# ymingxie/PARQ

Measured on AMD Instinct MI355X. Metric: decoder-iterations/sec (10 views, 256 queries, d=256), higher is better.
Workload: dtype f32 (cross-attention scores: fp16 hi.hi + MX-fp8 e4m3 cross terms; P V: fp16 probabilities and values with a self-consistent normaliser; fp32 accumulation — 4e-6..1.5e-5 from float64 at the outputs on the reference's fixtures, the reference's own fp32 run: 6e-5..1.4e-4; guarded: rows on too few keys

## Files before the change

parq_amd/csrc/api.hip:

```cpp
#include "../../include/parq_hip.h"
#include "common.hpp"

#include <cmath>
#include <cstdarg>
#include <cstdio>
#include <cstring>
#include <map>
#include <string>
#include <vector>

using namespace parq;

namespace {
constexpr float kPeakyL = 256.f;

thread_local char g_err[512] = "";

int fail(int code, const char* fmt, ...) {
    va_list ap;
    va_start(ap, fmt);
    vsnprintf(g_err, sizeof(g_err), fmt, ap);
    va_end(ap);
    return code;
}
// ... 434 lines not shown
            HIPCHK(half(L.cross_in_w, C, C, nullptr, A + L.n1_b, A + L.cross_in_b));
            HIPCHK(half(L.cross_out_w, C, C));
            HIPCHK(half(L.lin1_w, F, C, A + L.n2_w, A + L.n2_b, A + L.lin1_b)); HIPCHK(half(L.lin2_w, C, F));
        }
        HIPCHK(half(ar.pe2_w, C, C));
        if (c->nl == 1) HIPCHK(half(ar.heads1_w, c->NH1, C, A + ar.layers[0].n3_w, A + ar.layers[0].n3_b, A + ar.heads1_b));
        else HIPCHK(half(ar.heads1_w, c->NH1, C));
        HIPCHK(half(ar.heads2_w, C, C)); HIPCHK(half(ar.heads2_w + C * C, C, C));
    }
    c->derived_valid = true;
    return PARQ_OK;
}

struct ShardIO { int mask = 7; const float* in = nullptr; float* out = nullptr; int nranks = 1; };

int do_iterate(parq_ctx* c, const parq_scene* sc, float* wsp, const Workspace& ws, int layer_num, const float* ref,
               bool emb_valid, const parq_outputs* o, float* ref_out, hipStream_t s, int64_t shift = 0,
               float* emb_next = nullptr, bool train = false, const ShardIO& sh = ShardIO(), int64_t captured_row0 = -1,
               bool last_of_forward = false) {
    const void* const* ind = captured_row0 >= 0 ? reinterpret_cast<const void* const*>(wsp + ws.ind) : nullptr;
    const float* cam_in = ind ? wsp + ws.cam : sc->camera;
    const int64_t row0 = captured_row0 >= 0 ? captured_row0 : 0;
    float* wi = wsp + shift;
    const bool sharded = sh.mask != 7;
    if (!emb_next) emb_next = wi + ws.emb;
    const float dp = train ? c->drop_p : 0.f;
    const float* A = c->arena;
    const Arena& ar = c->ar;
    if (!train && !c->derived_valid) { const int rc = build_derived_weights(c, s); if (rc) return rc; }
    const float* TP = train ? nullptr : A + ar.tile_off;
    const bool h3 = !train && ar.half_off >= 0 && c->attn_mode != 0 && chain_h3_on();
    auto halfw = [&](LinearArgs& la, int64_t off, int fold = 0) {
        if (h3) {
            la.Wh = A + ar.half_off + off; la.wh_scale = A + ar.hscale_off + hscale_slot(off);
// ... 16 lines not shown
        return a;
    };
    auto cross_q_args = [&](bool fold) {
        LinearArgs a = lin(wi + ws.xa, C, A + L.cross_in_w, C, A + (fold ? L.cross_q_b2 : L.cross_in_b), wi + ws.qc, C, M, C, C);
        a.ln_gamma = A + L.n1_w; a.ln_beta = A + L.n1_b; a.ln_stats_out = wi + ws.ln1; a.norm_eps = eps;
        a.ldx2 = C; a.x2_ncols = C; a.Wp = TP ? TP + L.cross_in_w : nullptr; halfw(a, L.cross_in_w, 2);
        if (fold) { a.X2 = wi + ws.pe_h; a.W2 = A + L.cross_q_w2; a.W2p = TP ? TP + L.cross_q_w2 : nullptr; }
        else a.X2 = wi + ws.pos;
        return a;
    };
    static const bool fold_off = [] { const char* e = dev_env("PARQ_FOLD_POS"); return e && e[0] == '0'; }();
    const bool fold_pos = !train && !fold_off && chain_linear_supported(self_in_args(true), 1) && chain_linear_supported(cross_q_args(true), 1);
    static const int seams = [] { const char* e = dev_env("PARQ_FUSE_SEAMS"); return e ? atoi(e) : 1; }();
    const bool seam_ok = !train && !sharded && fold_pos && C == 256 && TP != nullptr && M % 16 == 0 && c->seam_fusion;

    if (sh.mask & 1) {
    if (!emb_valid) { Prof p(c, s, PARQ_PROF_OTHER); HIPCHK(launch_posemb(ref, A + ar.dim_t, M, wi + ws.emb, s)); }
    LinearArgs pe1 = lin(wi + ws.emb, 384, A + ar.pe0_w, 384, A + ar.pe0_b, wi + ws.pe_h, C, M, C, 384);
    pe1.relu = 1; pe1.Wp = TP ? TP + ar.pe0_w : nullptr;
    float* sample_out = sharded ? sh.out : wi + ws.tgt;
    float* sample_cnt = sharded ? sh.out + (int64_t)M * C : nullptr;
    static const bool fuse_off = [] { const char* e = dev_env("PARQ_FUSE_PE1_SAMPLE"); return e && e[0] == '0'; }();
    bool fused = false;
    if (!train && !fuse_off && !c->profiling) {
        const hipError_t e = launch_pe1_sample(pe1, sc->tokens, reinterpret_cast<const double*>(wsp + ws.T_cl), cam_in, ref, c->sb, B, sc->V,
                                               sc->h, sc->w, C, Q, sample_out, o->coord_pos, gn1, B * 8 * kGnSlots, sample_cnt, s, ind, row0 * 3,
                                               c->tok_type);
        if (e == hipSuccess) fused = true;
        else if (e != hipErrorNotSupported) return fail(PARQ_ERR_HIP, "launch_pe1_sample failed: %s", hipGetErrorString(e));
    }
    {
        Prof p(c, s, PARQ_PROF_LINEAR);
        if (!fused) HIPCHK(launch_linear(pe1, 1, s));
        if (!fold_pos) {
            LinearArgs a = lin(wi + ws.pe_h, C, A + ar.pe2_w, C, A + ar.pe2_b, wi + ws.pos, C, M, C, C);
            a.Wp = TP ? TP + ar.pe2_w : nullptr; halfw(a, ar.pe2_w);
            HIPCHK(launch_linear(a, 1, s));
        }
    }
    if (!fused) {
        Prof p(c, s, PARQ_PROF_PROJECT_SAMPLE);
        HIPCHK(launch_project_sample_f64(sc->tokens, reinterpret_cast<const double*>(wsp + ws.T_cl), cam_in, ref, c->sb,
                                         B, sc->V, sc->h, sc->w, C, Q, sample_out, o->coord_pos, gn1, B * 8 * kGnSlots, s, sample_cnt, ind, row0 * 3,
                                         c->tok_type));
    }
    if (sharded) HIPCHK(launch_shard_range_flag(c->cache_mode() && c->kind() == kF16 ? reinterpret_cast<const int*>(wsp + ws.flags) : nullptr,
                                                sh.out + (int64_t)M * C + M, s));
    }
    if (sh.mask & 2) {
    if (sharded) {
        Prof p(c, s, PARQ_PROF_PROJECT_SAMPLE);
        HIPCHK(launch_sample_finalize(sh.in, sh.in + (int64_t)M * C, M, C, wi + ws.tgt, s, sh.in + (int64_t)M * C + M,
                                      c->cache_mode() && c->kind() == kF16 ? reinterpret_cast<int*>(wsp + ws.flags) : nullptr));
    }
    {
        Prof p(c, s, PARQ_PROF_LINEAR);
        LinearArgs a = self_in_args(fold_pos);
        HIPCHK(launch_linear(a, 1, s));
    }
    FlashArgs fa;
    memset(&fa, 0, sizeof(fa));
    fa.B = B; fa.H = H; fa.Lq = Q; fa.dh = dh;
    fa.out = wi + ws.sa; fa.out_batch = (int64_t)Q * C; fa.out_row = C;
    {
        Prof p(c, s, PARQ_PROF_SELF_ATTN);
        static const bool self_one = [] { const char* e = dev_env("PARQ_SELF_ONE_LAUNCH"); return !(e && e[0] == '0'); }();
        if (dh <= 64 || (self_one && (dh == 128 || dh == 256) && Q <= 1024)) {
            HIPCHK(launch_self_attn(wi + ws.qkv, 3 * C, B, H, Q, dh, wi + ws.sa, C, s, train ? wi + ws.lse_s : nullptr, dp,
                                    c->site_seed(layer_num, 0)));
        } else {
            fa.q = wi + ws.qkv;         fa.q_batch = (int64_t)Q * 3 * C; fa.q_head = dh; fa.q_row = 3 * C;
            fa.k = wi + ws.qkv + C;     fa.k_batch = fa.q_batch; fa.k_head = dh; fa.k_row = 3 * C;
            fa.v = wi + ws.qkv + 2 * C; fa.v_batch = fa.q_batch; fa.v_head = dh; fa.v_row = 3 * C;
            fa.Lk = Q; fa.nsplit = ws.self_split;
            const int64_t lp = flash_lq_pad(Q);
            fa.o_part = wsp + ws.flash;
            fa.m_part = fa.o_part + (int64_t)B * H * fa.nsplit * dh * lp;
            fa.l_part = fa.m_part + (int64_t)B * H * fa.nsplit * lp;
            fa.lse = train ? wi + ws.lse_s : nullptr;
            fa.drop_p = dp; fa.drop_seed = c->site_seed(layer_num, 0);
            HIPCHK(launch_flash(fa, s));
            HIPCHK(launch_flash_merge(fa, s));
        }
    }
    fa.out = sharded ? sh.out : wi + ws.attn;
    fa.lse = sharded ? sh.out + (int64_t)M * C : (train ? wi + ws.lse_c : nullptr);
    fa.drop_p = dp; fa.drop_seed = c->site_seed(layer_num, 2);
    bool fused_q = false;
    {
        Prof p(c, s, PARQ_PROF_LINEAR);
        LinearArgs a = lin(wi + ws.sa, C, A + L.self_out_w, C, A + L.self_out_b, wi + ws.xa, C, M, C, C);
        a.R = wi + ws.tgt; a.ldr = C; a.Wp = TP ? TP + L.self_out_w : nullptr; halfw(a, L.self_out_w);
        a.drop_p = dp; a.drop_seed = c->site_seed(layer_num, 1);
        if (seam_ok && (seams & 1)) {
            a.lnp_out = reinterpret_cast<double*>(wi + ws.lnp1);
            a.lnp_flags = reinterpret_cast<unsigned*>(wsp + ws.seam_flags);
            a.lnp_epoch = c->next_epoch();
            SeamArgs q;
            memset(&q, 0, sizeof(q));
            q.X1 = wi + ws.sa; q.ldx1 = C; q.W1p = TP + L.qo_w;
            q.X2 = wi + ws.tgt; q.ldx2 = C; q.W2p = TP + L.qg_w;
            q.X3 = wi + ws.pe_h; q.ldx3 = C; q.W3p = TP + L.cross_q_w2;
            q.b1 = A + L.qu_b; q.srow = A + L.q_s; q.b2 = A + L.qv_b;
            q.Y = wi + ws.qc; q.ldy = C; q.M = M; q.N = C;
            q.part = a.lnp_out; q.flags = a.lnp_flags; q.epoch = a.lnp_epoch; q.nparts = C / 64; q.width = C; q.eps = eps;
            q.ln_out = wi + ws.ln1;
            q.err = reinterpret_cast<int*>(wsp + ws.flags);
            const hipError_t e = launch_seam_q(a, q, s);
            if (e == hipSuccess) fused_q = true;
            else if (e != hipErrorNotSupported) return fail(PARQ_ERR_HIP, "launch_seam_q failed: %s", hipGetErrorString(e));
            a.lnp_out = nullptr; a.lnp_flags = nullptr;
        }
        if (!fused_q) {
            HIPCHK(launch_linear(a, 1, s));
            a = cross_q_args(fold_pos);
            HIPCHK(launch_linear(a, 1, s));
        }
    }
    bool merged = false;
    {
        Prof p(c, s, PARQ_PROF_CROSS_ATTN);
        fa.q = wi + ws.qc; fa.q_batch = (int64_t)Q * C; fa.q_head = dh; fa.q_row = C;
        fa.Lk = (int)N; fa.nsplit = ws.cross_split;
        const int alt_phase = [] { const char* e = dev_env("PARQ_FLASH_ALT_PHASE"); return e && e[0] == '1' ? 1 : 0; }();
        fa.flags = ((layer_num + alt_phase) & 1) ? 2 : 0;
        const int64_t lp = flash_lq_pad(Q);
        fa.o_part = wsp + ws.flash;
        fa.m_part = fa.o_part + (int64_t)B * H * fa.nsplit * dh * lp;
        fa.l_part = fa.m_part + (int64_t)B * H * fa.nsplit * lp;
        if (c->cache_mode()) {
            const char* cache = reinterpret_cast<const char*>(wsp + ws.kvc) + (size_t)li * kvsplit_cache_bytes(B, c->vheads(), (int)N, c->terms());
// ... 29 lines not shown
                    { Prof pm(c, s, PARQ_PROF_MERGE); HIPCHK(launch_flash_merge(f8, s)); HIPCHK(launch_flash_merge(f3, s)); }
                    merged = true;
                }
            }
            else {
                if (c->attn_mode == 4 && !train && !sharded && H <= 16 && dh == 64) fa.head_min = reinterpret_cast<int*>(wsp + ws.flags) + 32;
                HIPCHK(launch_flash_split(fa, cache, s, c->terms(), c->kind()));
            }
        } else {
            const float* kv = wsp + ws.kv + (int64_t)li * B * 2 * N * C;
            fa.k = kv;                       fa.k_batch = 2 * N * C; fa.k_head = N * dh; fa.k_row = dh;
            fa.v = kv + (int64_t)H * N * dh; fa.v_batch = 2 * N * C; fa.v_head = N * dh; fa.v_row = dh;
            HIPCHK(launch_flash(fa, s));
        }
    }
    if (!merged) { Prof p(c, s, PARQ_PROF_MERGE); HIPCHK(launch_flash_merge(fa, s)); }
    }
    if (!(sh.mask & 4)) return PARQ_OK;
    if (sharded) {
        Prof p(c, s, PARQ_PROF_MERGE);
        const int64_t rec = (int64_t)M * C + (int64_t)B * H * flash_lq_pad(Q);
        HIPCHK(launch_attn_combine(sh.in, sh.nranks, rec, B, H, Q, flash_lq_pad(Q), dh, wi + ws.attn, s));
    }
    {
        Prof p(c, s, PARQ_PROF_LINEAR);
        LinearArgs a = lin(wi + ws.attn, C, A + L.cross_out_w, C, A + L.cross_out_b, wi + ws.xb, C, M, C, C);
        a.R = wi + ws.xa; a.ldr = C; a.rln_stats = wi + ws.ln1; a.rln_gamma = A + L.n1_w; a.rln_beta = A + L.n1_b; a.Wp = TP ? TP + L.cross_out_w : nullptr; halfw(a, L.cross_out_w);
        a.drop_p = dp; a.drop_seed = c->site_seed(layer_num, 3);
        if (last_of_forward && c->progress_word != nullptr) {
            a.pub_flags = reinterpret_cast<const int*>(wsp + ws.flags);
            a.pub_mirror = c->range_mirror; a.pub_word = c->progress_word;
            a.pub_epoch = reinterpret_cast<const int*>(wsp + ws.ind) + 14;
            a.pub_mask = (c->cache_mode() && c->kind() == kF16) ? ~0 : 4;
            a.pub_peaky = c->terms_for(N, false) == 8 ? 1 : 0;
        }
        HIPCHK(launch_linear(a, 1, s));
        a = lin(wi + ws.xb, C, A + L.lin1_w, C, A + L.lin1_b, wi + ws.ffn, F, M, F, C);
        a.ln_gamma = A + L.n2_w; a.ln_beta = A + L.n2_b; a.ln_stats_out = wi + ws.ln2; a.norm_eps = eps;
        a.relu = 1; a.Wp = TP ? TP + L.lin1_w : nullptr; halfw(a, L.lin1_w, 1);
        a.drop_p = dp; a.drop_seed = c->site_seed(layer_num, 4);
        HIPCHK(launch_linear(a, 1, s));
        a = lin(wi + ws.ffn, F, A + L.lin2_w, F, A + L.lin2_b, wi + ws.xc, C, M, C, F);
        a.R = wi + ws.xb; a.ldr = C; a.rln_stats = wi + ws.ln2; a.rln_gamma = A + L.n2_w; a.rln_beta = A + L.n2_b; a.Wp = TP ? TP + L.lin2_w : nullptr; halfw(a, L.lin2_w);
        a.drop_p = dp; a.drop_seed = c->site_seed(layer_num, 5);
        HIPCHK(launch_linear(a, 1, s));
        const int NH1 = c->NH1;
        a = lin(wi + ws.xc, C, A + ar.heads1_w, C, A + ar.heads1_b, wi + ws.h1, NH1, M, NH1, C);
        a.ln_gamma = A + L.n3_w; a.ln_beta = A + L.n3_b; a.norm_eps = eps;
        if (train) a.ln_stats_out = wi + ws.ln3;
        if (NH1 % 16 == 0) { a.Wp = TP ? TP + ar.heads1_w : nullptr; halfw(a, ar.heads1_w, c->nl == 1 ? 1 : 0); }
        a.gn_out_sums = gn1; a.gn_out_ncols = 2 * C; a.gn_out_group_cols = C; a.gn_out_rows_per_scene = Q; a.gn_out_ngroups = 2;
        HIPCHK(launch_linear(a, 1, s));
        if (train && c->deterministic) HIPCHK(launch_gn_moments_det(wi + ws.h1, NH1, C, 2, Q, B, gn1, s));
        a = lin(wi + ws.h1, NH1, A + ar.heads2_w, C, nullptr, wi + ws.h2, 2 * C, M, C, C);
        a.gn_sums = gn1; a.gn_gamma = A + ar.gn1_g; a.gn_beta = A + ar.gn1_b; a.norm_eps = eps;
        a.gn_rows_per_scene = Q; a.gn_ngroups = 2;
        a.gX = C; a.gW = (int64_t)C * C; a.gY = C; a.gGamma = C; a.Wp = TP ? TP + ar.heads2_w : nullptr; halfw(a, ar.heads2_w);
        a.gn_out_sums = gn2; a.gn_out_ncols = C; a.gn_out_group_cols = C; a.gn_out_rows_per_scene = Q; a.gn_out_ngroups = 2;
        HIPCHK(launch_linear(a, 2, s));
        if (train && c->deterministic) HIPCHK(launch_gn_moments_det(wi + ws.h2, 2 * C, C, 2, Q, B, gn2, s));
    }
    {
        Prof p(c, s, PARQ_PROF_OTHER);
        BoxDecodeArgs d;
        memset(&d, 0, sizeof(d));
        d.h1 = wi + ws.h1 + 2 * C; d.ld1 = c->NH1;
        d.h2 = wi + ws.h2; d.ld2 = 2 * C;
        d.gn_sums = gn2; d.gn_gamma = A + ar.gn2_g; d.gn_beta = A + ar.gn2_b;
        d.w3 = A + ar.heads3_w; d.b3 = A + ar.heads3_b; d.C = C; d.rows_per_scene = Q; d.eps = eps;
        d.ref = ref; d.mean_sizes = A + ar.mean_sizes; d.n_mean = c->cfg.num_mean_sizes; d.dim_t = A + ar.dim_t;
        d.poison = reinterpret_cast<const int*>(wsp + ws.flags);
        d.poison_mask = (c->cache_mode() && c->kind() == kF16) ? ~0 : 4;
        d.poison_mirror = (last_of_forward && c->progress_word != nullptr) ? nullptr : c->range_mirror;
        d.peaky = (!sharded && c->terms_for(N, train, train && bwd_reads_cache(c, ws)) == 8) ? reinterpret_cast<const int*>(wsp + ws.flags) + 1 : nullptr;
        d.peaky_poison = c->peaky_poison;
        d.sb = c->sb; d.M = M; d.ncls = c->ncls;
        d.logits = o->pred_logits; d.center = o->center_unnormalized; d.size = o->size_unnormalized;
        d.rot = o->ortho6d; d.prob = o->sem_cls_prob; d.ref_next = ref_out; d.emb_next = emb_next;
        d.ind = ind; d.out_row0 = row0;
        HIPCHK(launch_box_decode(d, s));
    }
    return PARQ_OK;
}


struct BwdIO {
    const float* g_logits; const float* g_center; const float* g_size; const float* g_rot;
    const float* center; const float* size;
};

int do_backward_transposes(parq_ctx* c, float* wsp, const Workspace& ws, int li, hipStream_t s) {
    const float* A = c->arena;
    const Arena& ar = c->ar;
    const LayerW& L = ar.layers[li];
    const int C = c->C, F = c->F, NH1 = c->NH1;
// ... 504 lines not shown
    const int64_t M = (int64_t)scene->B * h->Q;
    float* ra = wsp + ws.ref;
    float* rb = wsp + ws.ref_next;
    for (int k = 0; k < h->I; ++k) {
        parq_outputs o;
        memset(&o, 0, sizeof(o));
        if (!captured) {
            o.pred_logits = outs->pred_logits + k * M * h->ncls;
            o.center_unnormalized = outs->center_unnormalized + k * M * 3;
            o.size_unnormalized = outs->size_unnormalized + k * M * 3;
            o.ortho6d = outs->ortho6d + k * M * 6;
            o.sem_cls_prob = outs->sem_cls_prob + k * M * h->ncls;
            o.coord_pos = outs->coord_pos + k * M * 3;
        }
        const int rc = do_iterate(h, scene, wsp, ws, k, ra, true, &o, rb, s, 0, nullptr, false, ShardIO(),
                                  captured ? k * M : -1, k + 1 == h->I);
        if (rc) return rc;
        float* t = ra; ra = rb; rb = t;
    }
    h->ref_state = 0;
    h->prepared = false;
    return PARQ_OK;
}

static int forward_checks(parq_handle h, const parq_scene* scene, void* workspace, size_t workspace_bytes, const parq_outputs* outs, Workspace* ws) {
    if (!h || !workspace) return fail(PARQ_ERR_ARG, "NULL argument");
    if (!h->packed) return fail(PARQ_ERR_STATE, "parq_pack_weights must be called first");
    int rc = check_scene(h, scene);
    if (rc) return rc;
    rc = check_outs(outs);
    if (rc) return rc;
// ... 887 lines not shown
```

parq_amd/csrc/chain.hip:

```cpp
#include "common.hpp"
#include "sample_body.hpp"

namespace parq {

namespace {

typedef float f32x4v __attribute__((ext_vector_type(4)));

enum : int { kProNone = 0, kProLN = 1, kProGN = 2 };
enum : int { kResNone = 0, kResPlain = 1, kResLN = 2 };

template <int K, int NT, int PRO, int ADD2, bool BIAS, bool RELU, int RES, bool GNOUT, int NWV = 4, bool LNP = false>
__device__ __forceinline__ void chain_tile(const LinearArgs& a, const int block_x, const int block_y) {
    if (block_x == 0 && block_y == 0) publish_progress(a);
    static_assert(K % (16 * NWV) == 0 && NT >= 1 && NT <= 4 && (NWV == 4 || NWV == 8), "tile shape");
    constexpr int NCH = K / (16 * NWV);
    constexpr int CS = 16 * NWV;
    __shared__ __attribute__((aligned(16))) float red[NWV * NT * 4 * 64];
    __shared__ float lnred[NWV * 16 * 2];

    const int g = block_y;
    const int ntn = a.N / (16 * NT);
    int n0, m0;
    if (a.tile_map == 0) {
// ... 65 lines not shown
    }
    const int et = wave % NT;
    const int erow = lane >> 2, ec = (lane & 3) * 4;
    const int om = m0 + erow, on = n0 + et * 16 + ec;
    f32x4v e_bias = {0.f, 0.f, 0.f, 0.f}, e_r = {0.f, 0.f, 0.f, 0.f}, e_rg = {1.f, 1.f, 1.f, 1.f}, e_rb = {0.f, 0.f, 0.f, 0.f};
    float rmean = 0.f, rrstd = 1.f;
    if constexpr (BIAS) e_bias = *reinterpret_cast<const f32x4v*>(a.bias + g * a.gBias + on);
    if constexpr (RES != kResNone) e_r = *reinterpret_cast<const f32x4v*>(a.R + (int64_t)om * a.ldr + on);
    if constexpr (RES == kResLN) {
        e_rg = *reinterpret_cast<const f32x4v*>(a.rln_gamma + on);
        e_rb = *reinterpret_cast<const f32x4v*>(a.rln_beta + on);
        rmean = a.rln_stats[(int64_t)om * 2 + 0];
        rrstd = a.rln_stats[(int64_t)om * 2 + 1];
    }
    __builtin_amdgcn_sched_barrier(0);

    if constexpr (PRO == kProLN) {
        float sm = 0.f, sq = 0.f;
#pragma unroll
        for (int c = 0; c < NCH; ++c)
#pragma unroll
            for (int e = 0; e < 4; ++e) {
                const float d = av[c][e] - shift;
                sm += d;
                sq += d * d;
            }
        sm += __shfl_xor(sm, 16); sq += __shfl_xor(sq, 16);
        sm += __shfl_xor(sm, 32); sq += __shfl_xor(sq, 32);
        if (kq == 0) { lnred[(wave * 16 + li) * 2 + 0] = sm; lnred[(wave * 16 + li) * 2 + 1] = sq; }
        lds_barrier();
// ... 46 lines not shown
    if constexpr (ADD2 == 2) {
        if (n0 < a.x2_ncols) {
#pragma unroll
            for (int c = 0; c < NCH; ++c)
#pragma unroll
                for (int e = 0; e < 4; ++e)
#pragma unroll
                    for (int t = 0; t < NT; ++t) acc[t] = __builtin_amdgcn_mfma_f32_16x16x4f32(x2v[c][e], b2v[t][c][e], acc[t], 0, 0, 0);
        }
    }
#pragma unroll
    for (int t = 0; t < NT; ++t)
#pragma unroll
        for (int r = 0; r < 4; ++r) red[((wave * NT + t) * 4 + r) * 64 + lane] = acc[t][r];
    lds_barrier();
    if (wave >= NT) return;

    const int src = (wave * 4 + (erow & 3)) * 64 + (erow >> 2) * 16 + ec;
    f32x4v sum = *reinterpret_cast<const f32x4v*>(&red[src]);
#pragma unroll
    for (int w = 1; w < NWV; ++w) sum += *reinterpret_cast<const f32x4v*>(&red[src + w * NT * 256]);
    f32x4v y;
    double gs = 0.0, gq = 0.0;
#pragma unroll
    for (int e = 0; e < 4; ++e) {
        float v = sum[e] + e_bias[e];
        if constexpr (RELU) v = v > 0.f ? v : 0.f;
        if constexpr (RES == kResPlain) v += e_r[e];
        if constexpr (RES == kResLN) v += (e_r[e] - rmean) * rrstd * e_rg[e] + e_rb[e];
        y[e] = v;
        if constexpr (GNOUT || LNP) { gs += (double)v; gq += (double)v * (double)v; }
// ... 38 lines not shown
                const int cbs = a.gn_out_group_cols >> 4;
                const int rb = (m0 % a.gn_out_rows_per_scene) >> 4, cb = ((nt0 + g * a.N) % a.gn_out_group_cols) >> 4;
                const bool own = (a.gn_out_rows_per_scene >> 4) * cbs <= kGnSlots;
                const int slot = own ? rb * cbs + cb : (int)((block_x * NT + wave) % kGnSlots);
                double* dst = a.gn_out_sums + (((int64_t)(m0 / a.gn_out_rows_per_scene) * a.gn_out_ngroups + grp) * kGnSlots + slot) * 2;
                if (own) {
                    typedef double f64x2 __attribute__((ext_vector_type(2)));
                    *reinterpret_cast<f64x2*>(dst) = f64x2{gs, gq};
                } else {
                    atomicAdd(dst, gs);
                    atomicAdd(dst + 1, gq);
                }
            }
        }
    }
}

template <int K, int NT, int PRO, int ADD2, bool BIAS, bool RELU, int RES, bool GNOUT, int NWV = 4>
__global__ __launch_bounds__(NWV * 64) void chain_linear_kernel(LinearArgs a) {
    PARQ_TL_KERNEL(kTlLinear);
    chain_tile<K, NT, PRO, ADD2, BIAS, RELU, RES, GNOUT, NWV>(a, (int)blockIdx.x, (int)blockIdx.y);
}

struct SampleArgs {
    const void* tokens; const double* T_cl; const float* cam; const float* ref; ScaleBox sb; int V, h, w, C, Q;
    float* tgt; float* coord_pos; double* zero_f64; int zero_n; float* raw_count;
    const void* const* ind; int64_t coord_off;
};
template <int NCH, int TT = kTokF32>
__global__ __launch_bounds__(1024) void pe1_sample_kernel(LinearArgs a, SampleArgs sa, int n_lin) {
// ... 1037 lines not shown
    s.relu = a.relu != 0;
    s.res = a.R ? (a.rln_stats ? kResLN : kResPlain) : kResNone;
    s.gnout = a.gn_out_sums != nullptr;
    return s;
}

thread_local bool g_dry_run = false;

template <int K, int NT, int PRO, int ADD2, bool BIAS, bool RELU, int RES, bool GNOUT>
hipError_t go(const LinearArgs& a0, int groups, hipStream_t s) {
    if (g_dry_run) return hipSuccess;
    static const int map_env = [] { const char* e = dev_env("PARQ_CHAIN_MAP"); return e ? atoi(e) : 0; }();
    LinearArgs a = a0;
    a.tile_map = (map_env == 1 && a.M % 128 == 0) ? 1 : 0;
    const dim3 grid((unsigned)((a.N / (16 * NT)) * (a.M / 16)), groups, 1);
    hipLaunchKernelGGL((chain_linear_kernel<K, NT, PRO, ADD2, BIAS, RELU, RES, GNOUT>), grid, dim3(256), 0, s, a);
    return hipGetLastError();
}

template <int K, int NT, int PRO, int ADD2, bool BIAS, bool RELU, int RES, bool GNOUT>
hipError_t go8(const LinearArgs& a0, int groups, hipStream_t s) {
    if (g_dry_run) return hipSuccess;
    LinearArgs a = a0;
    a.tile_map = 0;
    const dim3 grid((unsigned)((a.N / (16 * NT)) * (a.M / 16)), groups, 1);
    hipLaunchKernelGGL((chain_linear_kernel<K, NT, PRO, ADD2, BIAS, RELU, RES, GNOUT, 8>), grid, dim3(512), 0, s, a);
    return hipGetLastError();
}

template <int K, int NT, int PRO, int ADD2, bool BIAS, bool RELU, int RES, bool GNOUT>
hipError_t go_stream(const LinearArgs& a0, int groups, hipStream_t s) {
    if (g_dry_run) return hipSuccess;
    LinearArgs a = a0;
    a.tile_map = 0;
    const dim3 grid((unsigned)((a.N / (16 * NT)) * (a.M / 16)), groups, 1);
    hipLaunchKernelGGL((chain_linear_stream_kernel<K, NT, PRO, ADD2, BIAS, RELU, RES, GNOUT>), grid, dim3(256), 0, s, a);
    return hipGetLastError();
}

template <int K, int NT, int PRO, int ADD2, bool BIAS, bool RELU, int RES, bool GNOUT>
// ... 210 lines not shown
}

hipError_t launch_pe1_sample(const LinearArgs& a_in, const void* tokens, const double* T_cl, const float* cam, const float* ref, ScaleBox sb,
                             int B, int V, int h, int w, int C, int Q, float* tgt, float* coord_pos, double* zero_f64, int zero_n,
                             float* raw_count, hipStream_t s, const void* const* ind, int64_t coord_off, int tok_type) {
    if (tok_type != kTokF32 && tok_type != kTokF16 && tok_type != kTokBF16) return hipErrorInvalidValue;
    if (!chain_linear_supported(a_in, 1)) return hipErrorNotSupported;
    const Sig g = sig_of(a_in);
    if (!(g.K == 384 && g.pro == kProNone && g.add2 == 0 && g.bias && g.relu && g.res == kResNone && !g.gnout)) return hipErrorNotSupported;
    if (C % 4 != 0 || C > 1024 || V <= 0 || V > 16) return hipErrorNotSupported;
    static const bool wp_off = [] { const char* e = dev_env("PARQ_CHAIN_WPACK"); return e && e[0] == '0'; }();
    LinearArgs a = a_in;
    if (wp_off || (a.Wp && (!al16(a.Wp) || a.ldw != a.K))) a.Wp = nullptr;
    a.tile_map = 0;
    const int n_lin = (a.N / 16) * (a.M / 16);
    const int nwv = V < 4 ? 4 : V;
    const size_t smem = (size_t)nwv * C * sizeof(float) + (size_t)nwv * sizeof(int) + (size_t)V * 32 + 16;
    SampleArgs sa{tokens, T_cl, cam, ref, sb, V, h, w, C, Q, tgt, coord_pos, zero_f64, zero_n, raw_count, ind, coord_off};
    const dim3 grid((unsigned)(n_lin + B * Q)), block(nwv * 64);
    const int nch = (C / 4 + 63) / 64;
    if (tok_type == kTokF16) launch_pe1_sample_t<kTokF16>(nch, grid, block, smem, s, a, sa, n_lin);
    else if (tok_type == kTokBF16) launch_pe1_sample_t<kTokBF16>(nch, grid, block, smem, s, a, sa, n_lin);
    else launch_pe1_sample_t<kTokF32>(nch, grid, block, smem, s, a, sa, n_lin);
    return hipGetLastError();
}

static bool fused_tile_ok(const LinearArgs& a) {
    return a.M % 16 == 0 && a.N == 256 && a.K == 256 && (a.ldx | a.ldw | a.y_row) % 4 == 0 && al16(a.X) && al16(a.W) && al16(a.Y) &&
           a.bias && al16(a.bias) && a.rows_per_batch == a.M && a.col_blk == a.N && !a.relu && !a.relu_mask && a.drop_p == 0.f && !a.X2 &&
           a.R && a.ldr % 4 == 0 && al16(a.R) && a.Wp && al16(a.Wp) && a.ldw == a.K && a.lnp_out && a.lnp_flags;
// ... 46 lines not shown
```

parq_amd/csrc/common.hpp:

```cpp
#pragma once

#include <hip/hip_runtime.h>
#include <stdint.h>
#include <stddef.h>
#include <stdlib.h>

namespace parq {

typedef float f32x4 __attribute__((ext_vector_type(4)));
typedef float f32x16 __attribute__((ext_vector_type(16)));

#ifdef PARQ_DEV_PROBES
inline const char* dev_env(const char* name) { return getenv(name); }
#else
inline const char* dev_env(const char*) { return nullptr; }
#endif

enum : int { kTlLinear = 1, kTlProjectSample = 2, kTlSelfAttn = 3, kTlFlashSplit = 4, kTlFlashMerge = 5, kTlBoxDecode = 6, kTlPosemb = 7,
             kTlKvProj = 8, kTlChain = 9 };
#ifdef PARQ_DEV_PROBES
static __device__ unsigned long long* parq_tl_buf = nullptr;
static __device__ unsigned int parq_tl_cap = 0;
struct TlStamp {
    unsigned long long t0, idx; int id;
// ... 231 lines not shown
        const uint2 r = reinterpret_cast<const uint2*>(row)[c4];
        if constexpr (TT == kTokF16) {
            const half2v a = __builtin_bit_cast(half2v, r.x), b = __builtin_bit_cast(half2v, r.y);
            return f32x4{(float)a[0], (float)a[1], (float)b[0], (float)b[1]};
        } else {
            return f32x4{bf16_bits_to_f32(r.x & 0xffffu), bf16_bits_to_f32(r.x >> 16), bf16_bits_to_f32(r.y & 0xffffu),
                         bf16_bits_to_f32(r.y >> 16)};
        }
    }
}

template <int KIND>
__device__ __forceinline__ f32x16 mfma16(half8 a, half8 b, f32x16 c) {
    if constexpr (KIND == kF16) return __builtin_amdgcn_mfma_f32_32x32x16_f16(a, b, c, 0, 0, 0);
    else return __builtin_amdgcn_mfma_f32_32x32x16_bf16(__builtin_bit_cast(bf16x8, a), __builtin_bit_cast(bf16x8, b), c, 0, 0, 0);
}

struct LinearArgs {
    const float* X;  int64_t ldx;
    const float* X2; int64_t ldx2;
    int x2_ncols;
    const float* W;  int64_t ldw;
    const float* bias;
    const float* R;  int64_t ldr;
    float* Y;
    int M, N, K;
    int relu;
    const float* relu_mask; int64_t ldmask;
    float mask_scale;
    float drop_p; uint32_t drop_seed;
// ... 1 lines not shown
    float norm_eps;
    const float* ln_gamma; const float* ln_beta; float* ln_stats_out;
    const float* rln_stats; const float* rln_gamma; const float* rln_beta;
    const double* gn_sums; const float* gn_gamma; const float* gn_beta;
    int gn_rows_per_scene; int gn_ngroups;
    double* gn_out_sums; int gn_out_ncols; int gn_out_group_cols; int gn_out_rows_per_scene; int gn_out_ngroups;
    int64_t gX, gW, gBias, gY, gGamma;
    const float* W2; const float* W2p;
    const float* Wp;
    const float* Wh; const float* wh_scale;
    const float* wh_bias; int wh_fold;
    int tile_map;
    double* lnp_out;
    unsigned* lnp_flags; unsigned lnp_epoch;
    const int* pub_flags; int* pub_mirror; int* pub_word; const int* pub_epoch; int pub_mask; int pub_peaky;
};
__device__ __forceinline__ void publish_progress(const LinearArgs& a) {
    if (a.pub_word != nullptr && blockIdx.x == 0 && blockIdx.y == 0 && threadIdx.x == 0) {
        const int f0 = a.pub_flags[0] & a.pub_mask, pk = a.pub_peaky ? a.pub_flags[1] : 0;
        const int bits = ((f0 & ~4) ? 1 : 0) | (f0 & 4) | (pk != 0 ? (2 | (pk << 8)) : 0);
        if (bits != 0 && a.pub_mirror != nullptr) __hip_atomic_fetch_or(a.pub_mirror, bits, __ATOMIC_RELAXED, __HIP_MEMORY_SCOPE_SYSTEM);
        __hip_atomic_store(a.pub_word, *a.pub_epoch, __ATOMIC_RELEASE, __HIP_MEMORY_SCOPE_SYSTEM);
    }
}
struct SeamArgs {
    const float* X1; int64_t ldx1; const float* W1p;
    const float* X2; int64_t ldx2; const float* W2p;
    const float* X3; int64_t ldx3; const float* W3p;
    const float* ln1_stats; const float* ln1_g; const float* ln1_b;
    const float* b1; const float* srow; const float* b2;
// ... 22 lines not shown
    int B, H, Lq, Lk, dh;
    int nsplit;
    float* o_part;
    float* m_part;
    float* l_part;
    float* out; int64_t out_batch, out_row;
    float defer_log2;
    float* lse;
    float drop_p; uint32_t drop_seed;
    int flags;
    int* peaky; float peaky_l;
    int* peaky_it; int* peaky_min;
    int* head_min;
    int nh; unsigned long long hmap;
    int64_t cache_head_bytes;
};
struct FlashHead { int b, h, bh; };
__device__ __forceinline__ FlashHead flash_head(const FlashArgs& a, int z) {
    FlashHead r;
    if (a.nh > 0) { r.b = z / a.nh; r.h = (int)((a.hmap >> (4 * (z - r.b * a.nh))) & 15ull); }
    else { r.b = z / a.H; r.h = z - r.b * a.H; }
    r.bh = r.b * a.H + r.h;
    return r;
}
inline int flash_launch_heads(const FlashArgs& a) { return a.nh > 0 ? a.nh : a.H; }
int flash_key_tile(int dh);
int flash_lq_pad(int Lq);
int flash_pick_nw(int B, int H, int Lq, int Lk, int dh, int num_cus);
int flash_pick_splits(int B, int H, int Lq, int Lk, int dh, int num_cus);
int device_num_cus();
// ... 207 lines not shown
```

parq_amd/csrc/flash.hip:

```cpp
#include "common.hpp"
#include <cstdlib>

namespace parq {

namespace {

template <int DH>
struct Tile {
    static constexpr int KT = DH <= 64 ? 64 : 32;
    static constexpr int ROW4 = DH / 4;
    static constexpr int SWZ = (ROW4 < 16 ? ROW4 : 16) - 1;
    static constexpr size_t lds_bytes() { return (size_t)2 * 2 * KT * DH * sizeof(float); }
};

template <int DH, int NW>
__global__ __launch_bounds__(NW * 64) void flash_f32_kernel(FlashArgs a) {
    using T = Tile<DH>;
    constexpr int KT = T::KT;
    constexpr int NT = NW * 64;
    constexpr int ROW4 = T::ROW4;
    constexpr int TILE4 = KT * ROW4;
    constexpr int LD4 = TILE4 / NT;
    static_assert(TILE4 % NT == 0, "tile must divide evenly over the workgroup");
    constexpr int NDT = DH / 32;
// ... 540 lines not shown
    const int half = threadIdx.x / (8 * DG);
    const int s_begin = half * SPT;
    const int64_t sstride = (int64_t)DH * Lq_pad;
    const float* o0 = a.o_part + (pb * DH + dg0 + dd) * (int64_t)Lq_pad + q0 + q4 * 4;

    float mloc[PER], lloc[PER];
#pragma unroll
    for (int i = 0; i < PER; ++i) {
        mloc[i] = a.m_part[(pb + td + i * 8) * Lq_pad + q];
        lloc[i] = a.l_part[(pb + td + i * 8) * Lq_pad + q];
    }
    f32x4 x[SPT];
#pragma unroll
    for (int u = 0; u < SPT; ++u) x[u] = *reinterpret_cast<const f32x4*>(o0 + (s_begin + u) * sstride);
    __builtin_amdgcn_sched_barrier(0);

    float mmax = -INFINITY;
#pragma unroll
    for (int i = 0; i < PER; ++i) mmax = fmaxf(mmax, mloc[i]);
    dsm[td * 32 + tq] = mmax;
    lds_barrier();
#pragma unroll
    for (int i = 0; i < 8; ++i) mmax = fmaxf(mmax, dsm[i * 32 + tq]);
    lds_barrier();
    float den = 0.f;
#pragma unroll
    for (int i = 0; i < PER; ++i) {
        const float w = __builtin_amdgcn_exp2f(mloc[i] - mmax);
        wsm[(td + i * 8) * 32 + tq] = w;
        den += w * lloc[i];
// ... 26 lines not shown
#pragma unroll
    for (int u = 0; u < SPT; ++u) acc += x[u] * *reinterpret_cast<const f32x4*>(&wsm[(s_begin + u) * 32 + q4 * 4]);
    *reinterpret_cast<f32x4*>(&part[(half * DG + dd) * 32 + q4 * 4]) = acc;
    lds_barrier();
    for (int idx = threadIdx.x; idx < 32 * DG; idx += 256) {
        const int qq = idx / DG;
        const int d = idx - qq * DG;
        float dn = 0.f;
#pragma unroll
        for (int i = 0; i < 8; ++i) dn += dsm[i * 32 + qq];
        float acc2 = 0.f;
#pragma unroll
        for (int g2 = 0; g2 < NG; ++g2) acc2 += part[(g2 * DG + d) * 32 + qq];
        a.out[(int64_t)b * a.out_batch + (int64_t)(q0 + qq) * a.out_row + h * DH + dg0 + d] = acc2 / dn;
    }
}

template <int DH, int NW>
hipError_t launch_one(const FlashArgs& a, hipStream_t s) {
    static DynLdsOnce once;
    const size_t lds = Tile<DH>::lds_bytes();
    if (hipError_t e = once.ensure(reinterpret_cast<const void*>(&flash_f32_kernel<DH, NW>), lds); e != hipSuccess) return e;
    dim3 grid(a.nsplit, ceil_div(a.Lq, 32 * NW), a.B * a.H);
    hipLaunchKernelGGL((flash_f32_kernel<DH, NW>), grid, dim3(NW * 64), lds, s, a);
    return hipGetLastError();
}

template <int DH>
hipError_t launch_dh(const FlashArgs& a, int nw, hipStream_t s) {
    switch (nw) {
// ... 4 lines not shown
            if constexpr (DH <= 64) return launch_one<DH, 8>(a, s);
            else return hipErrorInvalidValue;
        default: return hipErrorInvalidValue;
    }
}

template <int DH>
hipError_t merge_dh(const FlashArgs& a, hipStream_t s) {
    const size_t lds = ((size_t)a.nsplit * 32 + 8 * 32 + (size_t)2 * 16 * 32) * sizeof(float);
    static const int dg_env = [] { const char* e = dev_env("PARQ_MERGE_DG"); return e ? atoi(e) : 0; }();
    const int64_t wg16 = (int64_t)ceil_div(a.Lq, 32) * a.B * flash_launch_heads(a) * (DH / 16);
    const int dg = dg_env == 8 || dg_env == 16 ? dg_env : (wg16 < device_num_cus() ? 8 : 16);
    static const bool fixed_off = [] { const char* e = dev_env("PARQ_MERGE_FIXED"); return e && e[0] == '0'; }();
    if constexpr (DH == 64) {
        if (dg == 8 && a.nsplit == 64 && a.Lq % 32 == 0 && !fixed_off) {
            hipLaunchKernelGGL((flash_merge_fixed_kernel<DH, 8, 64>), dim3(a.Lq / 32, a.B * flash_launch_heads(a), DH / 8), dim3(256), 0, s, a);
            return hipGetLastError();
        }
    }
    if constexpr (DH == 256) {
        if (dg == 16 && a.nsplit == 32 && a.Lq % 32 == 0 && !fixed_off) {
            hipLaunchKernelGGL((flash_merge_fixed_kernel<DH, 16, 32>), dim3(a.Lq / 32, a.B * flash_launch_heads(a), DH / 16), dim3(256), 0, s, a);
            return hipGetLastError();
        }
    }
    if (dg == 8) {
        static DynLdsOnce once;
        if (hipError_t e = once.ensure(reinterpret_cast<const void*>(&flash_merge_kernel<DH, 8>), 96 * 1024); e != hipSuccess) return e;
        hipLaunchKernelGGL((flash_merge_kernel<DH, 8>), dim3(ceil_div(a.Lq, 32), a.B * flash_launch_heads(a), DH / 8), dim3(256), lds, s, a);
    } else {
        static DynLdsOnce once;
        if (hipError_t e = once.ensure(reinterpret_cast<const void*>(&flash_merge_kernel<DH, 16>), 96 * 1024); e != hipSuccess) return e;
        hipLaunchKernelGGL((flash_merge_kernel<DH, 16>), dim3(ceil_div(a.Lq, 32), a.B * flash_launch_heads(a), DH / 16), dim3(256), lds, s, a);
    }
    return hipGetLastError();
}

// ... 102 lines not shown
```

Before: 5893.

## Prefetch next stage weights into cache from preceding kernels in the chain

Adds a WarmArgs descriptor to linear and flash-merge kernels. Each block issues strided loads over the weight tiles the following kernel will read, spread across XCDs, and keeps the values live until the block ends so the loads are not eliminated. The aim is to hide the cold-cache weight fetch latency of each subsequent launch in the decoder iteration chain. The cost is extra memory traffic and registers in the current kernel. It also adds an env-gated PARQ_CHAIN_TWICE debug path that launches each kernel twice.

```diff
diff --git a/parq_amd/csrc/api.hip b/parq_amd/csrc/api.hip
--- a/parq_amd/csrc/api.hip
+++ b/parq_amd/csrc/api.hip
@@ -472,10 +472,12 @@
 
 struct ShardIO { int mask = 7; const float* in = nullptr; float* out = nullptr; int nranks = 1; };
 
+static bool chain_twice() { static const bool t = [] { const char* e = dev_env("PARQ_CHAIN_TWICE"); return e && e[0] == '1'; }(); return t; }
+#define HIPCHK_T(expr) do { HIPCHK(expr); if (chain_twice()) HIPCHK(expr); } while (0)
 int do_iterate(parq_ctx* c, const parq_scene* sc, float* wsp, const Workspace& ws, int layer_num, const float* ref,
                bool emb_valid, const parq_outputs* o, float* ref_out, hipStream_t s, int64_t shift = 0,
                float* emb_next = nullptr, bool train = false, const ShardIO& sh = ShardIO(), int64_t captured_row0 = -1,
-               bool last_of_forward = false) {
+               bool last_of_forward = false, bool warm = false) {
     const void* const* ind = captured_row0 >= 0 ? reinterpret_cast<const void* const*>(wsp + ws.ind) : nullptr;
     const float* cam_in = ind ? wsp + ws.cam : sc->camera;
     const int64_t row0 = captured_row0 >= 0 ? captured_row0 : 0;
@@ -522,10 +524,19 @@
     static const int seams = [] { const char* e = dev_env("PARQ_FUSE_SEAMS"); return e ? atoi(e) : 1; }();
     const bool seam_ok = !train && !sharded && fold_pos && C == 256 && TP != nullptr && M % 16 == 0 && c->seam_fusion;
 
+    static const int warm_env = [] { const char* e = dev_env("PARQ_CHAIN_WARM"); return e ? atoi(e) : 1; }();
+    const bool warm_on = warm && warm_env != 0 && TP != nullptr && !sharded;
+    auto warm_set = [&](WarmArgs& w, int64_t off0, int64_t n0, int64_t off1 = 0, int64_t n1 = 0) {
+        if (!warm_on) return;
+        w.p[0] = TP + off0; w.bytes[0] = (unsigned)(n0 * sizeof(float));
+        if (n1 > 0) { w.p[1] = TP + off1; w.bytes[1] = (unsigned)(n1 * sizeof(float)); }
+    };
+
     if (sh.mask & 1) {
     if (!emb_valid) { Prof p(c, s, PARQ_PROF_OTHER); HIPCHK(launch_posemb(ref, A + ar.dim_t, M, wi + ws.emb, s)); }
     LinearArgs pe1 = lin(wi + ws.emb, 384, A + ar.pe0_w, 384, A + ar.pe0_b, wi + ws.pe_h, C, M, C, 384);
     pe1.relu = 1; pe1.Wp = TP ? TP + ar.pe0_w : nullptr;
+    if (fold_pos) warm_set(pe1.warm, L.self_in_w2, 3 * (int64_t)C * C);
     float* sample_out = sharded ? sh.out : wi + ws.tgt;
     float* sample_cnt = sharded ? sh.out + (int64_t)M * C : nullptr;
     static const bool fuse_off = [] { const char* e = dev_env("PARQ_FUSE_PE1_SAMPLE"); return e && e[0] == '0'; }();
@@ -534,7 +545,7 @@
         const hipError_t e = launch_pe1_sample(pe1, sc->tokens, reinterpret_cast<const double*>(wsp + ws.T_cl), cam_in, ref, c->sb, B, sc->V,
                                                sc->h, sc->w, C, Q, sample_out, o->coord_pos, gn1, B * 8 * kGnSlots, sample_cnt, s, ind, row0 * 3,
                                                c->tok_type);
-        if (e == hipSuccess) fused = true;
+        if (e == hipSuccess) { fused = true; if (chain_twice()) (void)launch_pe1_sample(pe1, sc->tokens, reinterpret_cast<const double*>(wsp + ws.T_cl), cam_in, ref, c->sb, B, sc->V, sc->h, sc->w, C, Q, sample_out, o->coord_pos, gn1, B * 8 * kGnSlots, sample_cnt, s, ind, row0 * 3, c->tok_type); }
         else if (e != hipErrorNotSupported) return fail(PARQ_ERR_HIP, "launch_pe1_sample failed: %s", hipGetErrorString(e));
     }
     {
@@ -543,7 +554,7 @@
         if (!fold_pos) {
             LinearArgs a = lin(wi + ws.pe_h, C, A + ar.pe2_w, C, A + ar.pe2_b, wi + ws.pos, C, M, C, C);
             a.Wp = TP ? TP + ar.pe2_w : nullptr; halfw(a, ar.pe2_w);
-            HIPCHK(launch_linear(a, 1, s));
+            HIPCHK_T(launch_linear(a, 1, s));
         }
     }
     if (!fused) {
@@ -564,7 +575,8 @@
     {
         Prof p(c, s, PARQ_PROF_LINEAR);
         LinearArgs a = self_in_args(fold_pos);
-        HIPCHK(launch_linear(a, 1, s));
+        warm_set(a.warm, L.self_out_w, (int64_t)C * C, L.cross_in_w, (int64_t)C * C);
+        HIPCHK_T(launch_linear(a, 1, s));
     }
     FlashArgs fa;
     memset(&fa, 0, sizeof(fa));
@@ -574,7 +586,7 @@
         Prof p(c, s, PARQ_PROF_SELF_ATTN);
         static const bool self_one = [] { const char* e = dev_env("PARQ_SELF_ONE_LAUNCH"); return !(e && e[0] == '0'); }();
         if (dh <= 64 || (self_one && (dh == 128 || dh == 256) && Q <= 1024)) {
-            HIPCHK(launch_self_attn(wi + ws.qkv, 3 * C, B, H, Q, dh, wi + ws.sa, C, s, train ? wi + ws.lse_s : nullptr, dp,
+            HIPCHK_T(launch_self_attn(wi + ws.qkv, 3 * C, B, H, Q, dh, wi + ws.sa, C, s, train ? wi + ws.lse_s : nullptr, dp,
                                     c->site_seed(layer_num, 0)));
         } else {
             fa.q = wi + ws.qkv;         fa.q_batch = (int64_t)Q * 3 * C; fa.q_head = dh; fa.q_row = 3 * C;
@@ -588,7 +600,7 @@
             fa.lse = train ? wi + ws.lse_s : nullptr;
             fa.drop_p = dp; fa.drop_seed = c->site_seed(layer_num, 0);
             HIPCHK(launch_flash(fa, s));
-            HIPCHK(launch_flash_merge(fa, s));
+            HIPCHK_T(launch_flash_merge(fa, s));
         }
     }
     fa.out = sharded ? sh.out : wi + ws.attn;
@@ -600,6 +612,7 @@
         LinearArgs a = lin(wi + ws.sa, C, A + L.self_out_w, C, A + L.self_out_b, wi + ws.xa, C, M, C, C);
         a.R = wi + ws.tgt; a.ldr = C; a.Wp = TP ? TP + L.self_out_w : nullptr; halfw(a, L.self_out_w);
         a.drop_p = dp; a.drop_seed = c->site_seed(layer_num, 1);
+        if (fold_pos) warm_set(a.warm, L.cross_q_w2, (int64_t)C * C);
         if (seam_ok && (seams & 1)) {
             a.lnp_out = reinterpret_cast<double*>(wi + ws.lnp1);
             a.lnp_flags = reinterpret_cast<unsigned*>(wsp + ws.seam_flags);
@@ -615,14 +628,14 @@
             q.ln_out = wi + ws.ln1;
             q.err = reinterpret_cast<int*>(wsp + ws.flags);
             const hipError_t e = launch_seam_q(a, q, s);
-            if (e == hipSuccess) fused_q = true;
+            if (e == hipSuccess) { fused_q = true; if (chain_twice()) (void)launch_seam_q(a, q, s); }
             else if (e != hipErrorNotSupported) return fail(PARQ_ERR_HIP, "launch_seam_q failed: %s", hipGetErrorString(e));
             a.lnp_out = nullptr; a.lnp_flags = nullptr;
         }
         if (!fused_q) {
-            HIPCHK(launch_linear(a, 1, s));
+            HIPCHK_T(launch_linear(a, 1, s));
             a = cross_q_args(fold_pos);
-            HIPCHK(launch_linear(a, 1, s));
+            HIPCHK_T(launch_linear(a, 1, s));
         }
     }
     bool merged = false;
@@ -682,7 +695,7 @@
             HIPCHK(launch_flash(fa, s));
         }
     }
-    if (!merged) { Prof p(c, s, PARQ_PROF_MERGE); HIPCHK(launch_flash_merge(fa, s)); }
+    if (!merged) { Prof p(c, s, PARQ_PROF_MERGE); warm_set(fa.warm, L.cross_out_w, (int64_t)C * C, L.lin1_w, (int64_t)F * C); HIPCHK_T(launch_flash_merge(fa, s)); }
     }
     if (!(sh.mask & 4)) return PARQ_OK;
     if (sharded) {
@@ -695,6 +708,7 @@
         LinearArgs a = lin(wi + ws.attn, C, A + L.cross_out_w, C, A + L.cross_out_b, wi + ws.xb, C, M, C, C);
         a.R = wi + ws.xa; a.ldr = C; a.rln_stats = wi + ws.ln1; a.rln_gamma = A + L.n1_w; a.rln_beta = A + L.n1_b; a.Wp = TP ? TP + L.cross_out_w : nullptr; halfw(a, L.cross_out_w);
         a.drop_p = dp; a.drop_seed = c->site_seed(layer_num, 3);
+        warm_set(a.warm, L.lin2_w, (int64_t)C * F);
         if (last_of_forward && c->progress_word != nullptr) {
             a.pub_flags = reinterpret_cast<const int*>(wsp + ws.flags);
             a.pub_mirror = c->range_mirror; a.pub_word = c->progress_word;
@@ -702,30 +716,34 @@
             a.pub_mask = (c->cache_mode() && c->kind() == kF16) ? ~0 : 4;
             a.pub_peaky = c->terms_for(N, false) == 8 ? 1 : 0;
         }
-        HIPCHK(launch_linear(a, 1, s));
+        HIPCHK_T(launch_linear(a, 1, s));
         a = lin(wi + ws.xb, C, A + L.lin1_w, C, A + L.lin1_b, wi + ws.ffn, F, M, F, C);
         a.ln_gamma = A + L.n2_w; a.ln_beta = A + L.n2_b; a.ln_stats_out = wi + ws.ln2; a.norm_eps = eps;
         a.relu = 1; a.Wp = TP ? TP + L.lin1_w : nullptr; halfw(a, L.lin1_w, 1);
         a.drop_p = dp; a.drop_seed = c->site_seed(layer_num, 4);
-        HIPCHK(launch_linear(a, 1, s));
+        warm_set(a.warm, ar.heads1_w, (int64_t)c->NH1 * C);
+        HIPCHK_T(launch_linear(a, 1, s));
         a = lin(wi + ws.ffn, F, A + L.lin2_w, F, A + L.lin2_b, wi + ws.xc, C, M, C, F);
         a.R = wi + ws.xb; a.ldr = C; a.rln_stats = wi + ws.ln2; a.rln_gamma = A + L.n2_w; a.rln_beta = A + L.n2_b; a.Wp = TP ? TP + L.lin2_w : nullptr; halfw(a, L.lin2_w);
         a.drop_p = dp; a.drop_seed = c->site_seed(layer_num, 5);
-        HIPCHK(launch_linear(a, 1, s));
+        warm_set(a.warm, ar.heads2_w, 2 * (int64_t)C * C);
+        HIPCHK_T(launch_linear(a, 1, s));
         const int NH1 = c->NH1;
         a = lin(wi + ws.xc, C, A + ar.heads1_w, C, A + ar.heads1_b, wi + ws.h1, NH1, M, NH1, C);
         a.ln_gamma = A + L.n3_w; a.ln_beta = A + L.n3_b; a.norm_eps = eps;
         if (train) a.ln_stats_out = wi + ws.ln3;
         if (NH1 % 16 == 0) { a.Wp = TP ? TP + ar.heads1_w : nullptr; halfw(a, ar.heads1_w, c->nl == 1 ? 1 : 0); }
         a.gn_out_sums = gn1; a.gn_out_ncols = 2 * C; a.gn_out_group_cols = C; a.gn_out_rows_per_scene = Q; a.gn_out_ngroups = 2;
-        HIPCHK(launch_linear(a, 1, s));
+        if (!last_of_forward) warm_set(a.warm, ar.pe0_w, (int64_t)C * 384);
+        HIPCHK_T(launch_linear(a, 1, s));
         if (train && c->deterministic) HIPCHK(launch_gn_moments_det(wi + ws.h1, NH1, C, 2, Q, B, gn1, s));
         a = lin(wi + ws.h1, NH1, A + ar.heads2_w, C, nullptr, wi + ws.h2, 2 * C, M, C, C);
         a.gn_sums = gn1; a.gn_gamma = A + ar.gn1_g; a.gn_beta = A + ar.gn1_b; a.norm_eps = eps;
         a.gn_rows_per_scene = Q; a.gn_ngroups = 2;
         a.gX = C; a.gW = (int64_t)C * C; a.gY = C; a.gGamma = C; a.Wp = TP ? TP + ar.heads2_w : nullptr; halfw(a, ar.heads2_w);
         a.gn_out_sums = gn2; a.gn_out_ncols = C; a.gn_out_group_cols = C; a.gn_out_rows_per_scene = Q; a.gn_out_ngroups = 2;
-        HIPCHK(launch_linear(a, 2, s));
+        if (!last_of_forward) warm_set(a.warm, L.self_in_w, 3 * (int64_t)C * C);
+        HIPCHK_T(launch_linear(a, 2, s));
         if (train && c->deterministic) HIPCHK(launch_gn_moments_det(wi + ws.h2, 2 * C, C, 2, Q, B, gn2, s));
     }
     {
@@ -746,7 +764,7 @@
         d.logits = o->pred_logits; d.center = o->center_unnormalized; d.size = o->size_unnormalized;
         d.rot = o->ortho6d; d.prob = o->sem_cls_prob; d.ref_next = ref_out; d.emb_next = emb_next;
         d.ind = ind; d.out_row0 = row0;
-        HIPCHK(launch_box_decode(d, s));
+        HIPCHK_T(launch_box_decode(d, s));
     }
     return PARQ_OK;
 }
@@ -1281,7 +1299,7 @@
             o.coord_pos = outs->coord_pos + k * M * 3;
         }
         const int rc = do_iterate(h, scene, wsp, ws, k, ra, true, &o, rb, s, 0, nullptr, false, ShardIO(),
-                                  captured ? k * M : -1, k + 1 == h->I);
+                                  captured ? k * M : -1, k + 1 == h->I, true);
         if (rc) return rc;
         float* t = ra; ra = rb; rb = t;
     }
diff --git a/parq_amd/csrc/chain.hip b/parq_amd/csrc/chain.hip
--- a/parq_amd/csrc/chain.hip
+++ b/parq_amd/csrc/chain.hip
@@ -103,6 +103,8 @@
         rrstd = a.rln_stats[(int64_t)om * 2 + 1];
     }
     __builtin_amdgcn_sched_barrier(0);
+    WarmRegs wr;
+    warm_issue(a.warm, a.X, (unsigned)(block_y * (int)gridDim.x + block_x), (unsigned)tid, NWV * 64u, wr);
 
     if constexpr (PRO == kProLN) {
         float sm = 0.f, sq = 0.f;
@@ -179,7 +181,7 @@
 #pragma unroll
         for (int r = 0; r < 4; ++r) red[((wave * NT + t) * 4 + r) * 64 + lane] = acc[t][r];
     lds_barrier();
-    if (wave >= NT) return;
+    if (wave >= NT) { warm_sink(wr); return; }
 
     const int src = (wave * 4 + (erow & 3)) * 64 + (erow >> 2) * 16 + ec;
     f32x4v sum = *reinterpret_cast<const f32x4v*>(&red[src]);
@@ -248,6 +250,7 @@
             }
         }
     }
+    warm_sink(wr);
 }
 
 template <int K, int NT, int PRO, int ADD2, bool BIAS, bool RELU, int RES, bool GNOUT, int NWV = 4>
@@ -1315,6 +1318,7 @@
     LinearArgs a = a0;
     a.tile_map = (map_env == 1 && a.M % 128 == 0) ? 1 : 0;
     const dim3 grid((unsigned)((a.N / (16 * NT)) * (a.M / 16)), groups, 1);
+    a.warm.nblocks = grid.x * grid.y;
     hipLaunchKernelGGL((chain_linear_kernel<K, NT, PRO, ADD2, BIAS, RELU, RES, GNOUT>), grid, dim3(256), 0, s, a);
     return hipGetLastError();
 }
@@ -1325,6 +1329,7 @@
     LinearArgs a = a0;
     a.tile_map = 0;
     const dim3 grid((unsigned)((a.N / (16 * NT)) * (a.M / 16)), groups, 1);
+    a.warm.nblocks = grid.x * grid.y;
     hipLaunchKernelGGL((chain_linear_kernel<K, NT, PRO, ADD2, BIAS, RELU, RES, GNOUT, 8>), grid, dim3(512), 0, s, a);
     return hipGetLastError();
 }
@@ -1565,6 +1570,7 @@
     if (wp_off || (a.Wp && (!al16(a.Wp) || a.ldw != a.K))) a.Wp = nullptr;
     a.tile_map = 0;
     const int n_lin = (a.N / 16) * (a.M / 16);
+    a.warm.nblocks = (unsigned)n_lin;
     const int nwv = V < 4 ? 4 : V;
     const size_t smem = (size_t)nwv * C * sizeof(float) + (size_t)nwv * sizeof(int) + (size_t)V * 32 + 16;
     SampleArgs sa{tokens, T_cl, cam, ref, sb, V, h, w, C, Q, tgt, coord_pos, zero_f64, zero_n, raw_count, ind, coord_off};
diff --git a/parq_amd/csrc/common.hpp b/parq_amd/csrc/common.hpp
--- a/parq_amd/csrc/common.hpp
+++ b/parq_amd/csrc/common.hpp
@@ -269,6 +269,36 @@
 __device__ __forceinline__ f32x16 mfma16(half8 a, half8 b, f32x16 c) {
     if constexpr (KIND == kF16) return __builtin_amdgcn_mfma_f32_32x32x16_f16(a, b, c, 0, 0, 0);
     else return __builtin_amdgcn_mfma_f32_32x32x16_bf16(__builtin_bit_cast(bf16x8, a), __builtin_bit_cast(bf16x8, b), c, 0, 0, 0);
+}
+
+struct WarmArgs {
+    const void* p[2]; unsigned bytes[2];
+    unsigned nblocks;
+};
+constexpr int kWarmLoads = 6;
+typedef float warm_f32x4 __attribute__((ext_vector_type(4)));
+struct WarmRegs { warm_f32x4 v[2][kWarmLoads]; };
+__device__ __forceinline__ void warm_issue(const WarmArgs& w, const void* fallback, unsigned block, unsigned tid, unsigned nthreads, WarmRegs& r) {
+    const unsigned xcd_blocks = (w.nblocks + 7u - (block & 7u)) >> 3;
+    const unsigned first = ((block >> 3) * nthreads + tid) * 16u, step = xcd_blocks * nthreads * 16u;
+#pragma unroll
+    for (int j = 0; j < 2; ++j) {
+        const bool on = w.bytes[j] != 0;
+        const char* base = on ? static_cast<const char*>(w.p[j]) : static_cast<const char*>(fallback);
+        const unsigned last = on ? w.bytes[j] - 16u : 0u;
+#pragma unroll
+        for (int i = 0; i < kWarmLoads; ++i) {
+            const unsigned off = first + (unsigned)i * step;
+            r.v[j][i] = *reinterpret_cast<const warm_f32x4*>(base + (off < last ? off : last));
+        }
+    }
+    __builtin_amdgcn_sched_barrier(0);
+}
+__device__ __forceinline__ void warm_sink(const WarmRegs& r) {
+#pragma unroll
+    for (int j = 0; j < 2; ++j)
+#pragma unroll
+        for (int i = 0; i < kWarmLoads; ++i) asm volatile("" ::"v"(r.v[j][i]));
 }
 
 struct LinearArgs {
@@ -300,6 +330,7 @@
     double* lnp_out;
     unsigned* lnp_flags; unsigned lnp_epoch;
     const int* pub_flags; int* pub_mirror; int* pub_word; const int* pub_epoch; int pub_mask; int pub_peaky;
+    WarmArgs warm;
 };
 __device__ __forceinline__ void publish_progress(const LinearArgs& a) {
     if (a.pub_word != nullptr && blockIdx.x == 0 && blockIdx.y == 0 && threadIdx.x == 0) {
@@ -352,6 +383,7 @@
     int* head_min;
     int nh; unsigned long long hmap;
     int64_t cache_head_bytes;
+    WarmArgs warm;
 };
 struct FlashHead { int b, h, bh; };
 __device__ __forceinline__ FlashHead flash_head(const FlashArgs& a, int z) {
diff --git a/parq_amd/csrc/flash.hip b/parq_amd/csrc/flash.hip
--- a/parq_amd/csrc/flash.hip
+++ b/parq_amd/csrc/flash.hip
@@ -578,6 +578,8 @@
 #pragma unroll
     for (int u = 0; u < SPT; ++u) x[u] = *reinterpret_cast<const f32x4*>(o0 + (s_begin + u) * sstride);
     __builtin_amdgcn_sched_barrier(0);
+    WarmRegs wr;
+    warm_issue(a.warm, a.m_part, blockIdx.x + gridDim.x * (blockIdx.y + gridDim.y * blockIdx.z), threadIdx.x, 256u, wr);
 
     float mmax = -INFINITY;
 #pragma unroll
@@ -634,6 +636,7 @@
         for (int g2 = 0; g2 < NG; ++g2) acc2 += part[(g2 * DG + d) * 32 + qq];
         a.out[(int64_t)b * a.out_batch + (int64_t)(q0 + qq) * a.out_row + h * DH + dg0 + d] = acc2 / dn;
     }
+    warm_sink(wr);
 }
 
 template <int DH, int NW>
@@ -668,13 +671,17 @@
     static const bool fixed_off = [] { const char* e = dev_env("PARQ_MERGE_FIXED"); return e && e[0] == '0'; }();
     if constexpr (DH == 64) {
         if (dg == 8 && a.nsplit == 64 && a.Lq % 32 == 0 && !fixed_off) {
-            hipLaunchKernelGGL((flash_merge_fixed_kernel<DH, 8, 64>), dim3(a.Lq / 32, a.B * flash_launch_heads(a), DH / 8), dim3(256), 0, s, a);
+            FlashArgs aw = a;
+            aw.warm.nblocks = (unsigned)((a.Lq / 32) * a.B * flash_launch_heads(a) * (DH / 8));
+            hipLaunchKernelGGL((flash_merge_fixed_kernel<DH, 8, 64>), dim3(a.Lq / 32, a.B * flash_launch_heads(a), DH / 8), dim3(256), 0, s, aw);
             return hipGetLastError();
         }
     }
     if constexpr (DH == 256) {
         if (dg == 16 && a.nsplit == 32 && a.Lq % 32 == 0 && !fixed_off) {
-            hipLaunchKernelGGL((flash_merge_fixed_kernel<DH, 16, 32>), dim3(a.Lq / 32, a.B * flash_launch_heads(a), DH / 16), dim3(256), 0, s, a);
+            FlashArgs aw = a;
+            aw.warm.nblocks = (unsigned)((a.Lq / 32) * a.B * flash_launch_heads(a) * (DH / 16));
+            hipLaunchKernelGGL((flash_merge_fixed_kernel<DH, 16, 32>), dim3(a.Lq / 32, a.B * flash_launch_heads(a), DH / 16), dim3(256), 0, s, aw);
             return hipGetLastError();
         }
     }
```

New measurement: 5818, median of 2. 1.3% lower.
